# summmeer/session-based-news-recommendation

Hardware: AMD Instinct MI355X
Metric: sessions/sec TCAR train on Globo (synthetic globo fold) (higher is better)
Workload: dtype bf16 (logits GEMM on split-bf16 planes = 3 MFMAs per product, gradient GEMMs plain bf16; fp32 accumulate, fp32 master state)

## Files before the change

session-based-news-recommendation_amd/_lib.py:

```python
from __future__ import annotations

import ctypes as C
import os
import re
import subprocess
from typing import List

PKG_DIR = os.path.dirname(os.path.abspath(__file__))
CSRC = os.path.join(PKG_DIR, "csrc")
LIB_PATH = os.environ.get("TCAR_LIB") or os.path.join(PKG_DIR, "libtcar_hip.so")
SOURCES = ["gemm_f32.hip", "gemm_bf16.hip", "embed.hip", "pool.hip", "score.hip", "ce.hip", "optim.hip", "step.hip", "mha.hip",
           "sampler.hip", "norm.hip", "shard.hip", "segsum.hip", "query.hip", "select.hip", "cand.hip", "retrieve.hip",
           "buildid.hip"]
BUILD_ID_TU = "buildid.hip"


def _hipcc() -> str:
    for cand in (os.environ.get("HIPCC"), "/opt/rocm/bin/hipcc", "hipcc"):
        if cand and (os.path.isabs(cand) and os.path.exists(cand) or not os.path.isabs(cand)):
            return cand
    return "hipcc"


ABI_LAYERS = [("", "tcar_hip.h"), ("SERVE", "tcar_serve.h"), ("WINDOW", "tcar_window.h"), ("QUOTA", "tcar_quota.h"),
              ("SERVE_SHARD", "tcar_serve_shard.h"), ("CAND", "tcar_cand.h"), ("RETRIEVE", "tcar_retrieve.h"),
              ("RAGGED", "tcar_ragged.h")]


def _name(prefix: str, name: str) -> str:
    return prefix + "_" + name if prefix else name


for _prefix, _file in ABI_LAYERS:
    globals()[_name(_prefix, "HEADER")] = os.path.join(PKG_DIR, "..", "include", _file)
HEADERS = [os.path.join(CSRC, "tcar_common.h"), os.path.join(CSRC, "tcar_bf16_layout.h"), os.path.join(CSRC, "topk_rows.h"),
           os.path.join(CSRC, "ce_rows.h")] + \
    [globals()[_name(_prefix, "HEADER")] for _prefix, _ in ABI_LAYERS]
_ID_MARK = b"TCAR_BUILD_ID="


def _digest(paths) -> str:
    import hashlib
    h = hashlib.sha256()
    for p in paths:
        h.update(os.path.basename(p).encode() + b"\0")
        with open(p, "rb") as f:
            h.update(f.read())
    return h.hexdigest()[:32]


def source_build_id() -> str:
    import hashlib
    base = _digest([os.path.join(CSRC, s) for s in SOURCES] + HEADERS)
    return hashlib.sha256((base + "|" + " ".join(SAFE_FLAGS)).encode()).hexdigest()[:32]


def binary_build_id(path: str = LIB_PATH):
    try:
        with open(path, "rb") as f:
# ... 189 lines not shown
```

session-based-news-recommendation_amd/csrc/embed.hip:

```cpp
#include "tcar_common.h"
#include "tcar_bf16_layout.h"

typedef __attribute__((ext_vector_type(4))) __bf16 bf16x4_e;

namespace {

struct EmbArgs {
  tcar_dims_t d;
  tcar_tables_t tab;
  tcar_batch_t bt;
  TcarSignal sig;
  float* x_icp; float* x_pt; float* x_act; float* click_t;
  const float* dx_icp; const float* dx_pt; const float* dx_act; const float* dclick;
  tcar_grads_t g;
  const float* sq_g; long sq_len; float* sq_part; int n_gather;
};
struct EmbRagged { int R; const int32_t* rpos; };
__device__ __forceinline__ const EmbRagged& emb_ragged(const EmbRagged& r) { return r; }
__device__ __forceinline__ EmbRagged emb_ragged() { return EmbRagged{0, nullptr}; }


__device__ __forceinline__ int time_vocab(int k) {
  return k == 0 ? 13 : k == 1 ? 32 : k == 2 ? 8 : k == 3 ? 25 : k == 4 ? 61 : TCAR_DUR_VOCAB;
}
__device__ __forceinline__ int time_rowoff(int k) {
  return k == 0 ? 0 : k == 1 ? 13 : k == 2 ? 45 : k == 3 ? 53 : k == 4 ? 78 : 139;
}
constexpr int SMALL_ROWS = 150;

template <typename P>
__device__ __forceinline__ P pick5(P const (&arr)[5], int k) {
  return k == 0 ? arr[0] : k == 1 ? arr[1] : k == 2 ? arr[2] : k == 3 ? arr[3] : arr[4];
}

template <int NCH, class... RG>
__global__ __launch_bounds__(256) void gather_clip_fwd_kernel(const EmbArgs a, const RG... rg_) {
  constexpr bool RAGGED = sizeof...(RG) > 0;
  const EmbRagged& rg = emb_ragged(rg_...);
  const int lane = threadIdx.x & 63;
  const int wave_g = blockIdx.x * 4 + (threadIdx.x >> 6);
  const int nwaves = gridDim.x * 4;
  const int B = a.bt.B, T = a.bt.T, BT = RAGGED ? rg.R : B * T;
  const int ldh = a.d.ldh, ldt = a.d.ldt;
  const int ic = 2 * ldh, pt = 5 * ldt, ek = ic + pt, ct = 2 * ldt;
  const int sub = ldt >> 2;
  const int gpw = 64 / sub;
  const int grp = lane / sub, lin = lane - grp * sub;

  constexpr int R = 2;
  for (int row0 = wave_g; row0 < BT; row0 += R * nwaves) {
    float4 xi[R][NCH], xc[R][NCH], xp[R][NCH];
    bool live[R];
#pragma unroll
    for (int u = 0; u < R; ++u) {
      const int row = row0 + u * nwaves;
      live[u] = row < BT;
// ... 1431 lines not shown
```

session-based-news-recommendation_amd/csrc/gemm_f32.hip:

```cpp
#include "tcar_common.h"
#include "tcar_bf16_layout.h"
#include <stdlib.h>

typedef __attribute__((ext_vector_type(16))) float f32x16;

constexpr int BK = 32;
constexpr int MAXP = 10;
constexpr int MAXSEG = 3;

struct GemmProb {
  const float* A[MAXSEG];
  const float* B[MAXSEG];
  long lda[MAXSEG], ldb[MAXSEG];
  int K[MAXSEG];
  int nseg;
  float* C;
  long ldc;
  const float* bias;
  int M, N, act, beta;
  int ksplit, kchunk, mode;
  int mt, nt, wg_begin;
  int dact; const float* dact_y; long ld_dact_y; float* colsum;
  __bf16* plane_hi; __bf16* plane_lo; int plane_in32, plane_col0;
  __bf16* pack_hi; __bf16* pack_lo; int pack_in32, pack_c0, pack_c1;
// ... 387 lines not shown
          else *p = v;
          if (g.plane_hi) {
            const __bf16 h = (__bf16)v, l = (__bf16)(v - (float)h);
            const long o = kb32_off(row, gcol, g.plane_in32);
            g.plane_hi[o] = h;
            g.plane_lo[o] = l;
            if (packed) {
              const long po = kb32_off(row, pcol, g.pack_in32);
              g.pack_hi[po] = h;
              g.pack_lo[po] = l;
            }
          }
        }
      }
    }
  }
  if (g.dact && g.colsum) {
    csum += __shfl_xor(csum, 32);
    if (lane < 32 && col < g.N && csum != 0.f) atomicAdd(g.colsum + col, csum);
  }
  tcar_signal_done(ga.sig);
}

namespace {

template <int LA, int LB, int TM, int TN>
int launch_variant(const GroupArgs& ga, int nwg, hipStream_t st) {
  constexpr size_t lds = 2 * (TileGeo<LA, TM>::FLOATS + TileGeo<LB, TN>::FLOATS) * sizeof(float);
  TCAR_SET_LDS_ONCE((gemm_f32_kernel<LA, LB, TM, TN>), lds);
  TCAR_LAUNCH((gemm_f32_kernel<LA, LB, TM, TN>), dim3(nwg), dim3(256), lds, st, ga);
  TCAR_CHECK_LAUNCH();
  return TCAR_OK;
}

template <int LA, int LB>
int launch_layout(GroupArgs& ga, hipStream_t st) {
  long big = 0;
  for (int i = 0; i < ga.nprob; ++i)
    big += (long)((ga.p[i].M + 127) / 128) * ((ga.p[i].N + 127) / 128) * ga.p[i].ksplit;
  const int T = big >= 192 ? 128 : 64;
  int wg = 0;
  for (int i = 0; i < ga.nprob; ++i) {
    GemmProb& p = ga.p[i];
    p.mt = (p.M + T - 1) / T;
    p.nt = (p.N + T - 1) / T;
    p.wg_begin = wg;
// ... 100 lines not shown
}

extern "C" int tcar_gemm_x3_grouped(int layout, int nprob, const tcar_gemm_desc_t* descs, void* stream) {
  return tcar_gemm_x3_grouped_o(layout, nprob, descs, stream, nullptr);
}
int tcar_gemm_x3_grouped_o(int layout, int nprob, const tcar_gemm_desc_t* descs, void* stream, TcarOpt* o) {
  if (nprob <= 0) return TCAR_OK;
  if (layout < 0 || layout > 2 || nprob > MAXP || !descs) return TCAR_E_ARG;
  GroupArgs ga;
  ga.nprob = 0;
  for (int i = 0; i < nprob; ++i) {
    if (descs[i].M <= 0 || descs[i].N <= 0) continue;
    const int rc = fill_prob(ga.p[ga.nprob], layout, descs[i]);
    if (rc) return rc;
    ga.nprob++;
  }
  if (ga.nprob == 0) return TCAR_OK;
  hipStream_t st = (hipStream_t)stream;
  if (layout == 0) return launch_x3<0, 1>(ga, st, o);
  if (layout == 1) return launch_x3<0, 0>(ga, st, o);
  return launch_x3<1, 1>(ga, st, o);
}

extern "C" int tcar_gemm_f32(int layout, int M, int N, int K, const float* A, int64_t lda, const float* B, int64_t ldb,
                             float* C, int64_t ldc, const float* bias, int act, int beta, int splitk, void* stream) {
  if (M <= 0 || N <= 0 || K <= 0) return TCAR_OK;
  tcar_gemm_desc_t d = {};
  d.nseg = 1;
  d.A[0] = A; d.B[0] = B; d.lda[0] = lda; d.ldb[0] = ldb; d.K[0] = K;
  d.C = C; d.ldc = ldc; d.bias = bias; d.M = M; d.N = N; d.act = act; d.beta = beta; d.splitk = splitk; d.atomic = 0;
  return tcar_gemm_f32_grouped(layout, 1, &d, stream);
}

extern "C" int tcar_gemm_splitk_effective(int K, int splitk) {
  if (splitk < 1) splitk = 1;
  int kchunk = (K + splitk - 1) / splitk;
  kchunk = ((kchunk + BK - 1) / BK) * BK;
  return (K + kchunk - 1) / kchunk;
}

extern "C" int tcar_splitk_reduce(const float* slabs, int splitk, int M, int N, int64_t ld, float* out, void* stream) {
  if (M <= 0 || N <= 0) return TCAR_OK;
  if ((N & 3) || (ld & 3) || !tcar_aligned16(slabs) || !tcar_aligned16(out)) return TCAR_E_ARG;
  long total = (long)M * (N >> 2);
  int blocks = (int)((total + 255) / 256);
  if (blocks > 2048) blocks = 2048;
// ... 5 lines not shown
```

session-based-news-recommendation_amd/csrc/query.hip:

```cpp
#include "tcar_common.h"

namespace {
constexpr int QS = 4;
constexpr int CT = 128, H1 = 256, H2 = 512;
struct QMlpArgs {
  const float* click; const float* w1; const float* b1; const float* w2; const float* b2;
  float* q1; float* q;
  int B;
  TcarSignal sig;
};
__device__ __forceinline__ void st4_wt(float* p, float4 v, bool write_through) {
  if (write_through) st4_sc1(p, v);
  else st4(p, v);
}

__global__ __launch_bounds__(512) void query_mlp_kernel(const QMlpArgs a) {
  extern __shared__ __attribute__((aligned(16))) float lds[];
  float* clk = lds;
  float* q1s = clk + QS * CT;
  float* part = q1s + QS * H1;
  const int t = threadIdx.x;
  const int b0 = blockIdx.x * QS;
  const bool wt = a.sig.cnt != nullptr;
  const int cg = t & 63, kq = t >> 6;
  float4 w[16];
#pragma unroll
  for (int j = 0; j < 16; ++j) w[j] = ld4(a.w1 + (long)(kq * 16 + j) * H1 + cg * 4);
  if (t < QS * CT / 4) {
    const int s = t >> 5, c = t & 31;
    st4(clk + s * CT + c * 4, b0 + s < a.B ? ld4(a.click + (long)(b0 + s) * CT + c * 4) : zero4());
  }
  __syncthreads();
  {
    float4 acc[QS];
#pragma unroll
    for (int s = 0; s < QS; ++s) acc[s] = zero4();
#pragma unroll
    for (int j4 = 0; j4 < 4; ++j4) {
#pragma unroll
      for (int s = 0; s < QS; ++s) {
        const float4 c = *reinterpret_cast<const float4*>(clk + s * CT + kq * 16 + j4 * 4);
        acc[s] = fma4(w[j4 * 4 + 0], c.x, acc[s]);
        acc[s] = fma4(w[j4 * 4 + 1], c.y, acc[s]);
        acc[s] = fma4(w[j4 * 4 + 2], c.z, acc[s]);
        acc[s] = fma4(w[j4 * 4 + 3], c.w, acc[s]);
      }
    }
#pragma unroll
    for (int s = 0; s < QS; ++s) st4(part + (kq * QS + s) * H1 + cg * 4, acc[s]);
  }
  __syncthreads();
  if (t < QS * 64) {
    const int s = t >> 6;
// ... 135 lines not shown
  }
  tcar_signal_done(a.sig);
}
}

extern "C" int tcar_query_mlp_bwd(const tcar_dims_t* d, int B, const float* dq, const float* q1, const float* q1_w, const float* q2_w,
                                  float* dq1, float* dclick, void* stream) {
  return tcar_query_mlp_bwd_o(d, B, dq, q1, q1_w, q2_w, dq1, dclick, stream, nullptr);
}
int tcar_query_mlp_bwd_o(const tcar_dims_t* d, int B, const float* dq, const float* q1, const float* q1_w, const float* q2_w, float* dq1,
                         float* dclick, void* stream, TcarOpt* o) {
  if (!d || d->ldh != H1 || d->ldt * 2 != CT || B <= 0) return TCAR_E_ARG;
  if (!q1_w || !dq1 || !dclick || !tcar_aligned16(q1_w) || !tcar_aligned16(dq1)) return TCAR_E_ARG;
  if (dq && (!q1 || !q2_w || !tcar_aligned16(dq) || !tcar_aligned16(q2_w))) return TCAR_E_ARG;
  QBwdArgs a{};
  a.dq = dq; a.q1 = q1; a.w1 = q1_w; a.w2 = q2_w; a.dq1 = dq1; a.dclick = dclick; a.B = B;
  a.sig = tcar_sig(o);
  TCAR_LAUNCH(query_mlp_bwd_kernel, dim3((unsigned)((B + QS - 1) / QS)), dim3(512), 0, (hipStream_t)stream, a);
  TCAR_CHECK_LAUNCH();
  return TCAR_OK;
}

namespace {
}

extern "C" int tcar_query_mlp(const tcar_dims_t* d, int B, const float* click_t, const float* q1_w, const float* q1_b,
                              const float* q2_w, const float* q2_b, float* q1, float* q, void* stream) {
  return tcar_query_mlp_o(d, B, click_t, q1_w, q1_b, q2_w, q2_b, q1, q, stream, nullptr);
}
int tcar_query_mlp_o(const tcar_dims_t* d, int B, const float* click_t, const float* q1_w, const float* q1_b, const float* q2_w,
                     const float* q2_b, float* q1, float* q, void* stream, TcarOpt* o) {
  if (!d || d->ldh != H1 || d->ldt * 2 != CT || B <= 0) return TCAR_E_ARG;
  if (!click_t || !q1_w || !q1_b || !q2_w || !q2_b || !q1 || !q) return TCAR_E_ARG;
  if (!tcar_aligned16(click_t) || !tcar_aligned16(q1_w) || !tcar_aligned16(q1_b) || !tcar_aligned16(q2_w) || !tcar_aligned16(q2_b) ||
      !tcar_aligned16(q1) || !tcar_aligned16(q))
    return TCAR_E_ARG;
  QMlpArgs a{};
  a.click = click_t; a.w1 = q1_w; a.b1 = q1_b; a.w2 = q2_w; a.b2 = q2_b; a.q1 = q1; a.q = q; a.B = B;
  a.sig = tcar_sig(o);
  constexpr size_t lds = (size_t)(QS * CT + QS * H1 + 4 * QS * H2) * sizeof(float);
  TCAR_SET_LDS_ONCE(query_mlp_kernel, lds);
  TCAR_LAUNCH(query_mlp_kernel, dim3((unsigned)((B + QS - 1) / QS)), dim3(512), lds, (hipStream_t)stream, a);
  TCAR_CHECK_LAUNCH();
  return TCAR_OK;
}
```

session-based-news-recommendation_amd/csrc/step.hip:

```cpp
#include "tcar_common.h"
#include "../../include/tcar_serve_shard.h"
#include "../../include/tcar_cand.h"
#include "../../include/tcar_retrieve.h"
#include <stdlib.h>

static int env_int(const char* name, int dflt) {
  const char* v = getenv(name);
  return (v && *v) ? atoi(v) : dflt;
}
namespace {
struct Switch { const char* name; int32_t TcarTuning::*field; int dflt; };
const Switch kSwitches[] = {
    {"TCAR_BF16_TILE", &TcarTuning::bf16_tile, 0},          {"TCAR_BF16_KS", &TcarTuning::bf16_ks, 2},
    {"TCAR_WGRAD_KS", &TcarTuning::wgrad_ks, 1536},         {"TCAR_GATHER_BIG_ROWS", &TcarTuning::gather_big_rows, 16384},
    {"TCAR_MHA_MFMA", &TcarTuning::mha_mfma, 1},            {"TCAR_SORT_SCATTER", &TcarTuning::sort_scatter, 1},
    {"TCAR_DET_SMALL", &TcarTuning::det_small, 1},          {"TCAR_FUSED_CE", &TcarTuning::fused_ce, 2},
    {"TCAR_ONEHOT_TIME", &TcarTuning::onehot_time, 2},      {"TCAR_FLAG_FORK", &TcarTuning::flag_fork, 4095},
    {"TCAR_CE_FOLD", &TcarTuning::ce_fold, 1024},           {"TCAR_PROJ_SPLIT_ROWS", &TcarTuning::proj_split_rows, 1024},
};
static_assert(sizeof(kSwitches) / sizeof(kSwitches[0]) == 12 && sizeof(TcarTuning) == 12 * sizeof(int32_t), "twelve switches, one table");
}
const TcarTuning& tcar_tuning() {
  static const TcarTuning t = [] {
    TcarTuning x{};
// ... 238 lines not shown
  return onehot_bwd(c, bt) && tn(c).fused_ce >= 2 && c->ce_rowscale && c->aps16h && c->ce_form && 2 * c->d.ldh / 64 <= TCAR_ANCHOR_COLS;
}
}

extern "C" int tcar_step_forward(const tcar_ctx_t* c, const tcar_batch_t* bt, int refresh_time, void* stream) {
  return forward_impl(c, bt, refresh_time, stream, -1.f, false);
}

namespace {
struct ScoreOut {
  void* p_hi; void* p_lo; float* tclip; bool done;
  const int32_t* label = nullptr; const float* E = nullptr; int64_t ldE = 0; bool anchor_done = false;
};
template <class Hook>
int session_forward(const tcar_ctx_t* c, const tcar_batch_t* bt, const Geo& g, void* stream, bool planes, int ei, Hook hook,
                    ScoreOut* so = nullptr, const tcar_ragged_t* rg = nullptr) {
  const int B = bt->B, BT = rg ? rg->R : bt->B * bt->T;
  tcar_tables_t tab;
  tables_of(c, tab);
  const int fmask = tn(c).flag_fork;
  hipStream_t sq = (g.ldh == 256 && g.ldt == 64 && c->stream3 && c->ev3 && fork_host(c) && ((fmask >> FK_GATHER) & 1) &&
                    ((fmask >> FK_QUERY) & 1))
                       ? (hipStream_t)c->stream3 : nullptr;
  TcarOpt og = opt_of(c);
  if (sq) og.sig = fork_arm(c, FK_GATHER);
  if (ei >= 0) (void)hipEventRecord((hipEvent_t)c->ev_start[4 * c->ev_n + ei], (hipStream_t)stream);
  RET(tcar_gather_clip_fwd_rg(&c->d, &tab, bt, rg, c->x_icp, c->x_pt, c->x_act, c->click_t, stream, &og));
  if (ei >= 0) (void)hipEventRecord((hipEvent_t)c->ev_stop[4 * c->ev_n + ei], (hipStream_t)stream);
  const bool qside = sq && fork_commit(c, FK_GATHER, og);
  if (qside) {
    RET(fork_go(c, FK_GATHER, (hipStream_t)stream, sq, c->ev3));
    TcarOpt oq = opt_of(c);
    oq.sig = fork_arm(c, FK_QUERY);
    RET(tcar_query_mlp_o(&c->d, B, c->click_t, W(c, TCAR_V_Q1_W), W(c, TCAR_V_Q1_B), W(c, TCAR_V_Q2_W), W(c, TCAR_V_Q2_B), c->q1,
                         c->q, (void*)sq, &oq));
    if (!fork_commit(c, FK_QUERY, oq)) return TCAR_E_LAUNCH;
  }
  const bool qfused = qside || (g.ldh == 256 && g.ldt == 64 && c->scoring != 0);
  if (qfused && !qside)
    RET(tcar_query_mlp(&c->d, B, c->click_t, W(c, TCAR_V_Q1_W), W(c, TCAR_V_Q1_B), W(c, TCAR_V_Q2_W), W(c, TCAR_V_Q2_B), c->q1,
                       c->q, stream));
  const float* x_c = c->x_icp + g.ldh;
  const int n1 = units(g.ic) + units(g.ldh) + units(g.ldt), n2 = units(g.pt) + units(g.ldh);
  const int64_t stride = (int64_t)BT * g.ldh;
  const bool split = c->scoring && c->proj_slabs && c->proj_slab_floats >= (n1 + n2) * stride;
  const bool psplit = split && BT <= tn(c).proj_split_rows;
  TcarOpt op = opt_of(c);
  if (psplit) {
    float* s1 = c->proj_slabs;
    float* s2 = c->proj_slabs + n1 * stride;
    tcar_gemm_desc_t p[6];
    p[0] = prob1(BT, g.ldh, c->x_icp, g.ic, W(c, TCAR_V_M_WIN), g.ldh, g.ic, s1, g.ldh, nullptr, 0, 0, units(g.ic));
    p[1] = prob1(BT, g.ldh, x_c, g.ic, W(c, TCAR_V_M_WC), g.ldh, g.ldh, s1 + units(g.ic) * stride, g.ldh, nullptr, 0, 0, units(g.ldh));
    p[2] = prob1(BT, g.ldh, c->x_act, g.ldt, W(c, TCAR_V_M_WINT), g.ldh, g.ldt, s1 + (units(g.ic) + units(g.ldh)) * stride, g.ldh,
                 nullptr, 0, 0, units(g.ldt));
    p[3] = prob1(BT, g.ldh, c->x_pt, g.pt, W(c, TCAR_V_S_WIN), g.ldh, g.pt, s2, g.ldh, nullptr, 0, 0, units(g.pt));
    p[4] = prob1(BT, g.ldh, x_c, g.ic, W(c, TCAR_V_S_WC), g.ldh, g.ldh, s2 + units(g.pt) * stride, g.ldh, nullptr, 0, 0, units(g.ldh));
    p[5] = prob1(B, g.ldh, c->click_t, g.ct, W(c, TCAR_V_Q1_W), g.ldh, g.ct, c->q1, g.ldh, W(c, TCAR_V_Q1_B), 1);
    if (ei >= 0) (void)hipEventRecord((hipEvent_t)c->ev_start[3 * c->ev_n + ei], (hipStream_t)stream);
    RET(hook(0, &op));
    RET(small_gemm(c, 0, qfused ? 5 : 6, p, stream, &op));
    if (ei >= 0) (void)hipEventRecord((hipEvent_t)c->ev_stop[3 * c->ev_n + ei], (hipStream_t)stream);
  } else {
    tcar_gemm_desc_t p[3];
    p[0] = prob(BT, g.ldh, c->pre1, g.ldh);
    seg(p[0], c->x_icp, g.ic, W(c, TCAR_V_M_WIN), g.ldh, g.ic);
    seg(p[0], x_c, g.ic, W(c, TCAR_V_M_WC), g.ldh, g.ldh);
    seg(p[0], c->x_act, g.ldt, W(c, TCAR_V_M_WINT), g.ldh, g.ldt);
    p[1] = prob(BT, g.ldh, c->pre2, g.ldh);
    seg(p[1], c->x_pt, g.pt, W(c, TCAR_V_S_WIN), g.ldh, g.pt);
    seg(p[1], x_c, g.ic, W(c, TCAR_V_S_WC), g.ldh, g.ldh);
    p[2] = prob1(B, g.ldh, c->click_t, g.ct, W(c, TCAR_V_Q1_W), g.ldh, g.ct, c->q1, g.ldh, W(c, TCAR_V_Q1_B), 1);
    if (ei >= 0) (void)hipEventRecord((hipEvent_t)c->ev_start[3 * c->ev_n + ei], (hipStream_t)stream);
    RET(hook(0, &op));
    RET(small_gemm(c, 0, qfused ? 2 : 3, p, stream, &op));
    if (ei >= 0) (void)hipEventRecord((hipEvent_t)c->ev_stop[3 * c->ev_n + ei], (hipStream_t)stream);
  }
  RET(hook(1, &op));
  const TcarWait wq{};
  if (qside) {
    RET(fork_go(c, FK_QUERY, sq, (hipStream_t)stream, c->ev3));
  } else if (!qside && !qfused) {
    tcar_gemm_desc_t p = prob1(B, g.ic, c->q1, g.ldh, W(c, TCAR_V_Q2_W), g.ic, g.ldh, c->q, g.ic, W(c, TCAR_V_Q2_B), 2);
    RET(small_gemm(c, 0, 1, &p, stream));
  }
  RET(hook(2, &op));
  if (rg && psplit)
    RET(tcar_attn_pool_fwd_slabs_ragged(&c->d, B, rg, c->x_icp, c->x_pt, c->proj_slabs, n1, c->proj_slabs + n1 * stride, n2, stride,
                                        c->pre1, c->pre2, c->q, W(c, TCAR_V_M_WRES), W(c, TCAR_V_S_WRES), c->pooled, c->alpha, stream));
  else if (rg)
    RET(tcar_attn_pool_fwd_ragged(&c->d, B, rg, c->x_icp, c->x_pt, c->pre1, c->pre2, c->q, W(c, TCAR_V_M_WRES), W(c, TCAR_V_S_WRES),
                                  c->pooled, c->alpha, stream));
  else if (psplit)
    RET(tcar_attn_pool_fwd_slabs_w(&c->d, B, bt->T, c->x_icp, c->x_pt, c->proj_slabs, n1, c->proj_slabs + n1 * stride, n2, stride,
                                   c->pre1, c->pre2, c->q, W(c, TCAR_V_M_WRES), W(c, TCAR_V_S_WRES), c->pooled, c->alpha, stream, wq));
  else
    RET(tcar_attn_pool_fwd(&c->d, B, bt->T, c->x_icp, c->x_pt, c->pre1, c->pre2, c->q, W(c, TCAR_V_M_WRES),
                           W(c, TCAR_V_S_WRES), c->pooled, c->alpha, stream));
// ... 1163 lines not shown
```

session-based-news-recommendation_amd/csrc/tcar_common.h:

```cpp
#pragma once
#include <hip/hip_runtime.h>
#include <stdint.h>
#include <stdio.h>

#include "../../include/tcar_hip.h"
#include "../../include/tcar_ragged.h"

#define TCAR_CHECK_LAUNCH()                                   \
  do {                                                        \
    hipError_t e__ = hipGetLastError();                       \
    if (e__ != hipSuccess) {                                  \
      fprintf(stderr, "tcar: HIP error %d (%s) at %s:%d\n", (int)e__, hipGetErrorString(e__), __FILE__, __LINE__); \
      return TCAR_E_LAUNCH;                                   \
    }                                                         \
  } while (0)

#define TCAR_LAUNCH(...)                 \
  do {                                   \
    (void)hipGetLastError();             \
    hipLaunchKernelGGL(__VA_ARGS__);     \
  } while (0)

static inline bool tcar_aligned16(const void* p) { return (reinterpret_cast<uintptr_t>(p) & 15u) == 0; }

// ... 123 lines not shown
                     const float* q2_b, float* q1, float* q, void* stream, TcarOpt* o);
int tcar_attn_pool_bwd_slabs_o(const tcar_dims_t* d, int B, int T, const float* x_icp, const float* x_pt, const float* pre1,
                               const float* pre2, const float* q, const float* w_res1, const float* w_res2, const float* alpha,
                               const float* dpooled, int nd_ic, int nd_pt, int64_t dp_stride, float* dx_icp, float* dx_pt, float* dq,
                               float* dpre1, float* dpre2, float* gw_rows, void* stream, TcarOpt* o);
int tcar_query_mlp_bwd_o(const tcar_dims_t* d, int B, const float* dq, const float* q1, const float* q1_w, const float* q2_w, float* dq1,
                         float* dclick, void* stream, TcarOpt* o);
int tcar_small_tables_bwd_det_o(const tcar_dims_t* d, const tcar_tables_t* tab, const tcar_batch_t* bt, const float* dx_icp,
                                const float* dx_pt, const float* dx_act, const float* dclick, const tcar_grads_t* g, float* ws,
                                void* stream, TcarOpt* o, const float* cand_pc ,
                                int64_t ws_floats );
int tcar_cand_time_bwd_onehot_w(const tcar_dims_t* d, int B, const int32_t* inv_off, const float* qz, const float* dP,
                                const float* attout, int64_t ld_att, const float* tclip, float* ws, const tcar_grads_t* g, void* stream,
                                const TcarWait& wait_dp, int with_pieces);
inline const float* tcar_cand_pieces(const tcar_dims_t* d, const float* ws) { return ws + (long)139 * 32 * (d->ldt + 4); }
int tcar_sqnorm_o(const float* g, const tcar_segments_t* segs, float* sqn_dense, void* stream, TcarOpt* o);
int tcar_colsum_sqnorm_o(const float* g, const tcar_segments_t* segs, int ncs, const tcar_colsum_t* cs, float* sqn_dense, void* stream,
                         TcarOpt* o);
int tcar_attn_pool_fwd_slabs_w(const tcar_dims_t* d, int B, int T, const float* x_icp, const float* x_pt, const float* pre1_slabs,
                               int n1, const float* pre2_slabs, int n2, int64_t slab_stride, float* pre1, float* pre2, const float* q,
                               const float* w_res1, const float* w_res2, float* pooled, float* alpha, void* stream,
                               const TcarWait& wait_q);
int tcar_gemm_x3_grouped_o(int layout, int nprob, const tcar_gemm_desc_t* descs, void* stream, TcarOpt* o);
int tcar_gemm_bf16_perm_o(int layout, int M, int N, int K, const void* A_hi, const void* A_lo, int64_t a_inner, int64_t a_rows,
                          const void* B_hi, const void* B_lo, int64_t b_inner, int64_t b_rows, float* C, int64_t ldc, float* C2,
                          int64_t ldc2, int csplit, const int32_t* c2_perm, int c2_group, int nsplit, int splitk, void* stream,
                          TcarOpt* o);
int tcar_gemm_bf16_ce_o(int M, int N, int K, const void* A_hi, const void* A_lo, int64_t a_inner, int64_t a_rows, const void* B_hi,
                        const void* B_lo, int64_t b_inner, int64_t b_rows, int K1, const void* A2_hi, const void* A2_lo,
                        const void* B2_hi, int64_t inner2, void* p_hi, int64_t p_inner, int64_t p_rows, float* stats,
                        int64_t stats_floats, const int32_t* label, float* lab_logit, int nsplit, int32_t* group_width,
                        int32_t* ngroups, void* stream, TcarOpt* o);
int tcar_gemm_bf16_dx_onehot_o(int M, int N1, int K, const void* A_hi, int64_t a_inner, int64_t a_rows, const void* B_hi,
                               int64_t b_inner, int64_t b_rows, const void* B2_hi, int64_t inner2, float* C, int64_t ldc, int splitk,
                               void* stream, TcarOpt* o);
int tcar_gemm_bf16_de_qz_o(int M, int K, const void* A_hi, int64_t a_inner, int64_t a_rows, const void* B_hi, int64_t b_inner,
                           int64_t b_rows, int ldh, float* C, int64_t ldc, const int32_t* mwdhm, const int32_t* perm,
                           const float* tclip, float* qz, int tile, void* stream, TcarOpt* o);
int tcar_reduce_dact_onehot_o(const float* slabs, int splitk, int M, int ic, int64_t ld, const float* addend, int64_t ld_add,
                              const float* y, int64_t ldy, const float* tclip, float* out, int64_t ldo, float* dP, float* bias_grad0,
                              float* bias_grad1, void* stream, TcarOpt* o);
int tcar_neg_fwd_o(const tcar_dims_t* d, int B, int K, const float* E, const int32_t* neg, const float* attout, float weight,
                   float* neg_fb, float* coef, float* negpart, void* stream, TcarOpt* o);
int tcar_clip_adam_rest_keep_o(float* w2d, int64_t ldw, const float* g2d, float* m2d, float* v2d, int64_t rows, int32_t cols,
                               int32_t slot, const float* sqn_dense, const float* sqn_pieces, const int32_t* use_dense, float clip,
                               float lr_t, float b1, float b2, float eps, void* e16_hi, void* e16_lo, int64_t ld16,
// ... 83 lines not shown
```

Measured before the change: 1.237 million.

## Fuse embedding gather and norm-clip into the head projection GEMM

Adds a head kernel that gathers item, position and time embedding rows, applies per-row norm clipping in registers, writes the clipped activations and feeds them straight into the split-bf16 x3 MFMA projection GEMM. The click-time embedding gather moves into the query MLP kernel on the side stream. Together these remove the separate gather_clip kernel launch and its round trip of activations through global memory. The cost is redundant row-norm loads across N tiles, higher register pressure, and extra start-flag polling on the host to order the side-stream query work.

```diff
diff --git a/include/tcar_head.h b/include/tcar_head.h
--- /dev/null
+++ b/include/tcar_head.h
@@ -0,0 +1,23 @@
+#ifndef TCAR_HEAD_H
+#define TCAR_HEAD_H
+
+#include "tcar_hip.h"
+
+#ifdef __cplusplus
+extern "C" {
+#endif
+
+#define TCAR_HEAD_ABI_VERSION 1
+int tcar_head_abi_version(void);
+
+int tcar_head_gather_proj(const tcar_dims_t* d, const tcar_tables_t* tab, const tcar_batch_t* bt, int nprob,
+                          const tcar_gemm_desc_t* descs, float* x_icp, float* x_pt, float* x_act, void* stream);
+
+int tcar_query_mlp_click(const tcar_dims_t* d, int B, const int32_t* cw, const int32_t* ch, const float* week, const float* hour,
+                         float* click_t, const float* q1_w, const float* q1_b, const float* q2_w, const float* q2_b, float* q1, float* q,
+                         void* stream);
+
+#ifdef __cplusplus
+}
+#endif
+#endif
diff --git a/session-based-news-recommendation_amd/_lib.py b/session-based-news-recommendation_amd/_lib.py
--- a/session-based-news-recommendation_amd/_lib.py
+++ b/session-based-news-recommendation_amd/_lib.py
@@ -24,7 +24,7 @@
 
 ABI_LAYERS = [("", "tcar_hip.h"), ("SERVE", "tcar_serve.h"), ("WINDOW", "tcar_window.h"), ("QUOTA", "tcar_quota.h"),
               ("SERVE_SHARD", "tcar_serve_shard.h"), ("CAND", "tcar_cand.h"), ("RETRIEVE", "tcar_retrieve.h"),
-              ("RAGGED", "tcar_ragged.h")]
+              ("HEAD", "tcar_head.h"), ("RAGGED", "tcar_ragged.h")]
 
 
 def _name(prefix: str, name: str) -> str:
@@ -34,7 +34,7 @@
 for _prefix, _file in ABI_LAYERS:
     globals()[_name(_prefix, "HEADER")] = os.path.join(PKG_DIR, "..", "include", _file)
 HEADERS = [os.path.join(CSRC, "tcar_common.h"), os.path.join(CSRC, "tcar_bf16_layout.h"), os.path.join(CSRC, "topk_rows.h"),
-           os.path.join(CSRC, "ce_rows.h")] + \
+           os.path.join(CSRC, "ce_rows.h"), os.path.join(CSRC, "embed_rows.h")] + \
     [globals()[_name(_prefix, "HEADER")] for _prefix, _ in ABI_LAYERS]
 _ID_MARK = b"TCAR_BUILD_ID="
 
diff --git a/session-based-news-recommendation_amd/csrc/embed.hip b/session-based-news-recommendation_amd/csrc/embed.hip
--- a/session-based-news-recommendation_amd/csrc/embed.hip
+++ b/session-based-news-recommendation_amd/csrc/embed.hip
@@ -1,5 +1,6 @@
 #include "tcar_common.h"
 #include "tcar_bf16_layout.h"
+#include "embed_rows.h"
 
 typedef __attribute__((ext_vector_type(4))) __bf16 bf16x4_e;
 
@@ -20,18 +21,10 @@
 __device__ __forceinline__ EmbRagged emb_ragged() { return EmbRagged{0, nullptr}; }
 
 
-__device__ __forceinline__ int time_vocab(int k) {
-  return k == 0 ? 13 : k == 1 ? 32 : k == 2 ? 8 : k == 3 ? 25 : k == 4 ? 61 : TCAR_DUR_VOCAB;
-}
 __device__ __forceinline__ int time_rowoff(int k) {
   return k == 0 ? 0 : k == 1 ? 13 : k == 2 ? 45 : k == 3 ? 53 : k == 4 ? 78 : 139;
 }
 constexpr int SMALL_ROWS = 150;
-
-template <typename P>
-__device__ __forceinline__ P pick5(P const (&arr)[5], int k) {
-  return k == 0 ? arr[0] : k == 1 ? arr[1] : k == 2 ? arr[2] : k == 3 ? arr[3] : arr[4];
-}
 
 template <int NCH, class... RG>
 __global__ __launch_bounds__(256) void gather_clip_fwd_kernel(const EmbArgs a, const RG... rg_) {
diff --git a/session-based-news-recommendation_amd/csrc/embed_rows.h b/session-based-news-recommendation_amd/csrc/embed_rows.h
--- /dev/null
+++ b/session-based-news-recommendation_amd/csrc/embed_rows.h
@@ -0,0 +1,18 @@
+#pragma once
+#include "tcar_common.h"
+
+__device__ __forceinline__ int time_vocab(int k) {
+  return k == 0 ? 13 : k == 1 ? 32 : k == 2 ? 8 : k == 3 ? 25 : k == 4 ? 61 : TCAR_DUR_VOCAB;
+}
+template <typename P>
+__device__ __forceinline__ P pick5(P const (&arr)[5], int k) {
+  return k == 0 ? arr[0] : k == 1 ? arr[1] : k == 2 ? arr[2] : k == 3 ? arr[3] : arr[4];
+}
+__device__ __forceinline__ int item_row(int id, int n_items) { return clampi(id, 1, n_items) - 1; }
+__device__ __forceinline__ int small_row(int k, int id) {
+  if (k == 5 && (id >= TCAR_DUR_VOCAB || id < 0)) return -1;
+  return clampi(id, 0, time_vocab(k) - 1);
+}
+__device__ __forceinline__ float row256_sumsq(float v0, float v1, float v2, float v3) {
+  return group_sum((v0 + v2) + (v1 + v3), 16);
+}
diff --git a/session-based-news-recommendation_amd/csrc/gemm_f32.hip b/session-based-news-recommendation_amd/csrc/gemm_f32.hip
--- a/session-based-news-recommendation_amd/csrc/gemm_f32.hip
+++ b/session-based-news-recommendation_amd/csrc/gemm_f32.hip
@@ -1,5 +1,7 @@
 #include "tcar_common.h"
 #include "tcar_bf16_layout.h"
+#include "embed_rows.h"
+#include "../../include/tcar_head.h"
 #include <stdlib.h>
 
 typedef __attribute__((ext_vector_type(16))) float f32x16;
@@ -433,6 +435,269 @@
   tcar_signal_done(ga.sig);
 }
 
+enum { XSRC_ICP = 0, XSRC_C = 1, XSRC_ACT = 2, XSRC_PT = 3 };
+struct HeadArgs {
+  GroupArgs ga;
+  tcar_tables_t tab;
+  const int32_t* seq; const int32_t* pub[5]; const int32_t* gap;
+  int T, n_items;
+  float* x_icp; float* x_pt; float* x_act;
+  unsigned char asrc[MAXP][4];
+  unsigned* start_flag; unsigned start_epoch;
+};
+static_assert(sizeof(HeadArgs) <= 4096, "kernel arguments");
+__device__ __forceinline__ void x3_name4(v4f (&a)[4]) {
+  asm volatile("" : "+v"(a[0]), "+v"(a[1]), "+v"(a[2]), "+v"(a[3]) : : "memory");
+}
+template <int N>
+__device__ __forceinline__ void x3_wait12(v4f (&a)[4], v4f (&p)[4], v4f (&b)[4]) {
+  asm volatile("s_waitcnt vmcnt(%12)"
+               : "+v"(a[0]), "+v"(a[1]), "+v"(a[2]), "+v"(a[3]), "+v"(p[0]), "+v"(p[1]), "+v"(p[2]), "+v"(p[3]), "+v"(b[0]), "+v"(b[1]),
+                 "+v"(b[2]), "+v"(b[3])
+               : "n"(N) : "memory");
+}
+__device__ __forceinline__ float4 x3_f4(const v4f& v) { return make_float4(v.x, v.y, v.z, v.w); }
+__device__ __forceinline__ float x3_sq(const v4f& v) { const float4 x = x3_f4(v); return dot4(x, x); }
+
+template <int XD>
+__global__ __launch_bounds__(256) void gemm_x3_head_kernel(const HeadArgs ha) {
+  constexpr int XK = 64, X3_PLANE = X3<XK>::PLANE, NV = 4;
+  constexpr int LDH = 256, LDT = 64, IC = 2 * LDH, PT = 5 * LDT, EK = IC + PT;
+  static_assert(X3<XK>::NV == NV, "four 16-byte loads per thread, operand and stage");
+  extern __shared__ __attribute__((aligned(16))) float smem_f[];
+  char* smem = reinterpret_cast<char*>(smem_f);
+  const GroupArgs& ga = ha.ga;
+  const int tid = threadIdx.x, wave = tid >> 6, lane = tid & 63;
+  if (ha.start_flag && blockIdx.x == 0 && tid == 0)
+    __hip_atomic_store(ha.start_flag, ha.start_epoch, __ATOMIC_RELAXED, __HIP_MEMORY_SCOPE_AGENT);
+  const int wm = wave >> 1, wn = wave & 1;
+  const int nwg = gridDim.x, bid = blockIdx.x;
+  const int xcd = bid & 7, q = nwg >> 3, r = nwg & 7;
+  int id = (xcd < r ? xcd * (q + 1) : r * (q + 1) + (xcd - r) * q) + (bid >> 3);
+  int pi = 0;
+#pragma unroll
+  for (int i = 1; i < MAXP; ++i) pi += (id >= ga.wg0[i]) ? 1 : 0;
+  const GemmProb& g = ga.p[pi];
+  id -= g.wg_begin;
+  const int tiles = g.mt * g.nt;
+  const int split = id / tiles;
+  id -= split * tiles;
+  int tm, tn;
+  if (g.mt <= g.nt) { tn = id / g.mt; tm = id - tn * g.mt; } else { tm = id / g.nt; tn = id - tm * g.nt; }
+  const int m0 = tm * 64, n0 = tn * 64;
+
+  const int ks = split * g.kchunk;
+  int cst[MAXSEG + 1], src[MAXSEG];
+  cst[0] = 0;
+  bool need_ip = false, need_c = false, need_pt = false, need_act = false;
+#pragma unroll
+  for (int sg = 0; sg < MAXSEG; ++sg) {
+    int n = 0;
+    src[sg] = ha.asrc[pi][sg];
+    if (sg < g.nseg) {
+      const int ke = min(g.K[sg], ks + g.kchunk);
+      n = ke > ks ? (ke - ks + XK - 1) / XK : 0;
+      if (n > 0) {
+        need_ip = need_ip || (src[sg] == XSRC_ICP && ks < LDH);
+        need_c = need_c || src[sg] == XSRC_C || (src[sg] == XSRC_ICP && ke > LDH);
+        need_pt = need_pt || src[sg] == XSRC_PT;
+        need_act = need_act || src[sg] == XSRC_ACT;
+      }
+    }
+    cst[sg + 1] = cst[sg] + n;
+  }
+  const int total = cst[MAXSEG];
+  const int b_rmax0 = (g.N + 3) & ~3;
+
+  const int j4 = (tid & 15) * 4, rb0 = tid >> 4;
+  bool rok[NV];
+  int itm[NV], pos[NV], dw[NV], sid[NV][5];
+#pragma unroll
+  for (int i = 0; i < NV; ++i) {
+    const int gr = m0 + rb0 + 16 * i;
+    rok[i] = gr < g.M;
+    const int rw = rok[i] ? gr : m0;
+    itm[i] = 0; dw[i] = 0;
+#pragma unroll
+    for (int k = 0; k < 5; ++k) sid[i][k] = 0;
+    pos[i] = rw % ha.T;
+    if (need_ip || need_c) itm[i] = item_row(ha.seq[rw], ha.n_items);
+    if (need_act) dw[i] = small_row(5, ha.gap[rw]);
+    if (need_pt) {
+#pragma unroll
+      for (int k = 0; k < 5; ++k) sid[i][k] = small_row(k, ha.pub[k][rw]);
+    }
+  }
+
+  auto stage_seg = [&](int s) { return min((s >= cst[1] ? 1 : 0) + (s >= cst[2] ? 1 : 0), g.nseg - 1); };
+  auto seg_src = [&](int sg) { return sg == 0 ? src[0] : sg == 1 ? src[1] : src[2]; };
+  auto load_stage = [&](int s, v4f (&ra)[NV], v4f (&rp)[NV], v4f (&rb)[NV], unsigned& ma, unsigned& mb) {
+    const int sg = stage_seg(s);
+    const int k0 = ks + (s - cst[sg]) * XK;
+    const int ke = min(g.K[sg], ks + g.kchunk);
+    const int sr = seg_src(sg);
+    const bool live = k0 < ke;
+    const bool ip = sr == XSRC_ICP && k0 < LDH, ct = sr == XSRC_C || (sr == XSRC_ICP && k0 >= LDH);
+    const int col = (sr == XSRC_ICP ? (k0 & (LDH - 1)) : k0) + (ct ? LDH : 0);
+    const int tb = sr == XSRC_ACT ? 5 : (k0 >> 6);
+    const float* tp = tb >= 5 ? ha.tab.dur : pick5(ha.tab.time, tb);
+    ma = 0;
+#pragma unroll
+    for (int i = 0; i < NV; ++i) {
+      const int sm = tb >= 5 ? dw[i] : pick5(sid[i], tb);
+      const bool ok = rok[i] && live && (ip || ct || sm >= 0);
+      const float* pe = ha.tab.E + (long)itm[i] * EK + col + j4;
+      const float* ps = tp + (long)(sm < 0 ? 0 : sm) * LDT + j4;
+      const float* pp = ha.tab.pos + (long)pos[i] * LDH + col + j4;
+      ra[i] = gload16_hidden(ok ? ((ip || ct) ? pe : ps) : ha.tab.pos);
+      rp[i] = gload16_hidden((ok && ip) ? pp : ha.tab.pos);
+      ma |= ok ? (1u << i) : 0u;
+    }
+    const long ldb = g.ldb[sg];
+    mb = x3_load<1, XK>(g.B[sg], ldb, n0, min((int)ldb, b_rmax0), k0, ke, tid, rb);
+  };
+
+  f32x16 acc;
+#pragma unroll
+  for (int e = 0; e < 16; ++e) acc[e] = 0.f;
+  v4f ra[XD][NV], rp[XD][NV], rb[XD][NV];
+  unsigned ma[XD], mb[XD];
+#pragma unroll
+  for (int d = 0; d < XD; ++d) load_stage(d, ra[d], rp[d], rb[d], ma[d], mb[d]);
+
+  float s_i[NV], s_p[NV], s_c[NV];
+#pragma unroll
+  for (int i = 0; i < NV; ++i) { s_i[i] = 1.f; s_p[i] = 1.f; s_c[i] = 1.f; }
+  auto row_norms = [&](const float* base, long stride, const int (&rowi)[NV], float (&out)[NV]) {
+    v4f x[NV][4];
+#pragma unroll
+    for (int i = 0; i < NV; ++i)
+#pragma unroll
+      for (int c = 0; c < 4; ++c) x[i][c] = gload16_hidden(base + (long)rowi[i] * stride + 64 * c + j4);
+    asm volatile("s_waitcnt vmcnt(0)" ::: "memory");
+#pragma unroll
+    for (int i = 0; i < NV; ++i) {
+      x3_name4(x[i]);
+      out[i] = clip_scale(row256_sumsq(x3_sq(x[i][0]), x3_sq(x[i][1]), x3_sq(x[i][2]), x3_sq(x[i][3])));
+    }
+  };
+  if constexpr (XD == 2) {
+    if (need_ip || need_c) {
+      const int oc = ((((ks & (LDH - 1)) >> 7) ^ 1) << 7) + (need_c ? LDH : 0) + j4;
+      v4f x[NV][2], y[NV][2];
+#pragma unroll
+      for (int i = 0; i < NV; ++i)
+#pragma unroll
+        for (int c = 0; c < 2; ++c) {
+          x[i][c] = gload16_hidden(ha.tab.E + (long)itm[i] * EK + oc + 64 * c);
+          if (need_ip) y[i][c] = gload16_hidden(ha.tab.pos + (long)pos[i] * LDH + oc + 64 * c);
+        }
+      asm volatile("s_waitcnt vmcnt(0)" ::: "memory");
+      x3_name4(ra[0]);
+      x3_name4(ra[1]);
+      x3_name4(rp[0]);
+      x3_name4(rp[1]);
+#pragma unroll
+      for (int i = 0; i < NV; ++i) {
+        asm volatile("" : "+v"(x[i][0]), "+v"(x[i][1]) : : "memory");
+        const float sa = clip_scale(group_sum((x3_sq(ra[0][i]) + x3_sq(x[i][0])) + (x3_sq(ra[1][i]) + x3_sq(x[i][1])), 16));
+        if (need_ip) {
+          asm volatile("" : "+v"(y[i][0]), "+v"(y[i][1]) : : "memory");
+          s_i[i] = sa;
+          s_p[i] = clip_scale(group_sum((x3_sq(rp[0][i]) + x3_sq(y[i][0])) + (x3_sq(rp[1][i]) + x3_sq(y[i][1])), 16));
+        } else {
+          s_c[i] = sa;
+        }
+      }
+    }
+  } else if (need_ip) {
+    v4f x[NV][4], y[NV][4];
+#pragma unroll
+    for (int i = 0; i < NV; ++i)
+#pragma unroll
+      for (int c = 0; c < 4; ++c) {
+        x[i][c] = gload16_hidden(ha.tab.E + (long)itm[i] * EK + 64 * c + j4);
+        y[i][c] = gload16_hidden(ha.tab.pos + (long)pos[i] * LDH + 64 * c + j4);
+      }
+    asm volatile("s_waitcnt vmcnt(0)" ::: "memory");
+#pragma unroll
+    for (int i = 0; i < NV; ++i) {
+      x3_name4(x[i]);
+      x3_name4(y[i]);
+      s_i[i] = clip_scale(row256_sumsq(x3_sq(x[i][0]), x3_sq(x[i][1]), x3_sq(x[i][2]), x3_sq(x[i][3])));
+      s_p[i] = clip_scale(row256_sumsq(x3_sq(y[i][0]), x3_sq(y[i][1]), x3_sq(y[i][2]), x3_sq(y[i][3])));
+    }
+  }
+  if (XD != 2 && need_c) row_norms(ha.tab.E + LDH, EK, itm, s_c);
+#pragma unroll
+  for (int d = 0; d < XD; ++d) {
+    x3_name4(ra[d]);
+    x3_name4(rp[d]);
+    x3_name4(rb[d]);
+  }
+
+  const bool keep = tn == 0;
+#pragma unroll 1
+  for (int base = 0; base < total; base += XD) {
+#pragma unroll
+    for (int d = 0; d < XD; ++d) {
+      const int s = base + d;
+      __syncthreads();
+      x3_wait12<(XD - 1) * 3 * NV>(ra[d], rp[d], rb[d]);
+      const int sg = stage_seg(s);
+      const int k0 = ks + (s - cst[sg]) * XK;
+      const int sr = seg_src(sg);
+      const bool ip = sr == XSRC_ICP && k0 < LDH, ct = sr == XSRC_C || (sr == XSRC_ICP && k0 >= LDH);
+      const int tb = sr == XSRC_ACT ? 5 : (k0 >> 6);
+      float* xo = sr == XSRC_ICP ? ha.x_icp + k0 + j4 : sr == XSRC_ACT ? ha.x_act + j4 : ha.x_pt + tb * LDT + j4;
+      const long xld = sr == XSRC_ICP ? IC : sr == XSRC_ACT ? LDT : PT;
+      const bool st = keep && sr != XSRC_C && s < total;
+#pragma unroll
+      for (int i = 0; i < NV; ++i) {
+        const bool ok = (ma[d] >> i) & 1u;
+        const float4 a = ok ? x3_f4(ra[d][i]) : zero4();
+        float4 v;
+        if (ip) v = fma4(a, s_i[i], scale4(x3_f4(rp[d][i]), s_p[i]));
+        else if (ct) v = scale4(a, s_c[i]);
+        else v = scale4(a, clip_scale(group_sum(dot4(a, a), 16)));
+        ra[d][i] = v4f{v.x, v.y, v.z, v.w};
+        if (st && rok[i]) st4(xo + (long)(m0 + rb0 + 16 * i) * xld, ok ? v : zero4());
+      }
+      x3_store<0, XK>(smem, smem + X3_PLANE, tid, ra[d], ma[d]);
+      x3_store<1, XK>(smem + 2 * X3_PLANE, smem + 3 * X3_PLANE, tid, rb[d], mb[d]);
+      __syncthreads();
+      load_stage(s + XD, ra[d], rp[d], rb[d], ma[d], mb[d]);
+      const int left = min(g.K[sg], ks + g.kchunk) - k0;
+      const int nsub = s < total ? (min(XK, left + 15) >> 4) : 0;
+#pragma unroll 2
+      for (int u = 0; u < nsub; ++u) {
+        const xbf16x8 ah = x3_frag<0, XK>(smem, wm * 32, u, lane), bh = x3_frag<1, XK>(smem + 2 * X3_PLANE, wn * 32, u, lane);
+        const xbf16x8 al = x3_frag<0, XK>(smem + X3_PLANE, wm * 32, u, lane), bl = x3_frag<1, XK>(smem + 3 * X3_PLANE, wn * 32, u, lane);
+        acc = __builtin_amdgcn_mfma_f32_32x32x16_bf16(al, bh, acc, 0, 0, 0);
+        acc = __builtin_amdgcn_mfma_f32_32x32x16_bf16(ah, bl, acc, 0, 0, 0);
+        acc = __builtin_amdgcn_mfma_f32_32x32x16_bf16(ah, bh, acc, 0, 0, 0);
+      }
+    }
+  }
+  asm volatile("s_waitcnt vmcnt(0)" ::: "memory");
+  float* Cs = g.C + (g.mode == 1 ? (long)split * g.M * g.ldc : 0L);
+  const bool wt = ga.sig.cnt != nullptr;
+  const int col = n0 + wn * 32 + (lane & 31);
+  if (col < g.N) {
+#pragma unroll
+    for (int e = 0; e < 16; ++e) {
+      const int row = m0 + wm * 32 + (e & 3) + 8 * (e >> 2) + 4 * (lane >> 5);
+      if (row < g.M) {
+        float* p = Cs + (long)row * g.ldc + col;
+        const float v = acc[e] + 0.f;
+        if (wt) __hip_atomic_store(p, v, __ATOMIC_RELAXED, __HIP_MEMORY_SCOPE_AGENT);
+        else *p = v;
+      }
+    }
+  }
+  tcar_signal_done(ga.sig);
+}
+
 namespace {
 
 template <int LA, int LB, int TM, int TN>
@@ -579,6 +844,78 @@
   return launch_x3<1, 1>(ga, st, o);
 }
 
+namespace {
+template <int XD>
+int launch_head(const HeadArgs& ha, int wg, hipStream_t st) {
+  constexpr size_t lds = 4 * X3<64>::PLANE;
+  TCAR_SET_LDS_ONCE((gemm_x3_head_kernel<XD>), lds);
+  TCAR_LAUNCH((gemm_x3_head_kernel<XD>), dim3(wg), dim3(256), lds, st, ha);
+  TCAR_CHECK_LAUNCH();
+  return TCAR_OK;
+}
+}
+
+extern "C" int tcar_head_abi_version(void) { return TCAR_HEAD_ABI_VERSION; }
+extern "C" int tcar_head_gather_proj(const tcar_dims_t* d, const tcar_tables_t* tab, const tcar_batch_t* bt, int nprob,
+                                     const tcar_gemm_desc_t* descs, float* x_icp, float* x_pt, float* x_act, void* stream) {
+  return tcar_head_gather_proj_o(d, tab, bt, nprob, descs, x_icp, x_pt, x_act, stream, nullptr);
+}
+int tcar_head_gather_proj_o(const tcar_dims_t* d, const tcar_tables_t* tab, const tcar_batch_t* bt, int nprob, const tcar_gemm_desc_t* descs,
+                            float* x_icp, float* x_pt, float* x_act, void* stream, TcarOpt* o) {
+  if (!d || !tab || !bt || !descs || d->ldh != 256 || d->ldt != 64 || d->n_items < 1) return TCAR_E_ARG;
+  if (bt->B <= 0 || bt->T <= 0 || bt->T > TCAR_POS_VOCAB || nprob < 1 || nprob > MAXP) return TCAR_E_ARG;
+  if (!tab->E || !tab->pos || !tab->dur || !bt->seq || !bt->gap || !x_icp || !x_pt || !x_act) return TCAR_E_ARG;
+  for (int k = 0; k < 5; ++k)
+    if (!tab->time[k] || !bt->pub[k] || !tcar_aligned16(tab->time[k])) return TCAR_E_ARG;
+  if (!tcar_aligned16(tab->E) || !tcar_aligned16(tab->pos) || !tcar_aligned16(tab->dur) || !tcar_aligned16(x_icp) || !tcar_aligned16(x_pt) ||
+      !tcar_aligned16(x_act))
+    return TCAR_E_ARG;
+  const long rows = (long)bt->B * bt->T;
+  const int ldh = 256, ldt = 64, ic = 2 * ldh, pt = 5 * ldt;
+  HeadArgs ha{};
+  GroupArgs& ga = ha.ga;
+  ga.nprob = 0;
+  int wg = 0, max_stages = 0;
+  bool oneshot = true;
+  for (int i = 0; i < nprob; ++i) {
+    const tcar_gemm_desc_t& ds = descs[i];
+    if (ds.M != rows || ds.bias || ds.act || ds.beta || ds.dact || ds.plane_hi || ds.pack_hi || ds.atomic) return TCAR_E_ARG;
+    GemmProb& p = ga.p[ga.nprob];
+    const int rc = fill_prob(p, 0, ds);
+    if (rc) return rc;
+    if (p.kchunk & 63) return TCAR_E_ARG;
+    int n = 0;
+    for (int s = 0; s < ds.nseg; ++s) {
+      int src;
+      if (ds.A[s] == x_icp && ds.lda[s] == ic && ds.K[s] == ic) src = XSRC_ICP;
+      else if (ds.A[s] == x_icp + ldh && ds.lda[s] == ic && ds.K[s] == ldh) src = XSRC_C;
+      else if (ds.A[s] == x_act && ds.lda[s] == ldt && ds.K[s] == ldt) src = XSRC_ACT;
+      else if (ds.A[s] == x_pt && ds.lda[s] == pt && ds.K[s] == pt) src = XSRC_PT;
+      else return TCAR_E_ARG;
+      ha.asrc[ga.nprob][s] = (unsigned char)src;
+      if ((src == XSRC_ICP || src == XSRC_C) && p.kchunk != 128) oneshot = false;
+      n += ((p.K[s] < p.kchunk ? p.K[s] : p.kchunk) + 63) / 64;
+    }
+    max_stages = n > max_stages ? n : max_stages;
+    p.mt = (p.M + 63) / 64;
+    p.nt = (p.N + 63) / 64;
+    p.wg_begin = wg;
+    ga.wg0[ga.nprob] = wg;
+    wg += p.mt * p.nt * p.ksplit;
+    ga.nprob++;
+  }
+  for (int i = ga.nprob; i < MAXP; ++i) ga.wg0[i] = 0x7fffffff;
+  ha.tab = *tab;
+  ha.seq = bt->seq; ha.gap = bt->gap;
+  for (int k = 0; k < 5; ++k) ha.pub[k] = bt->pub[k];
+  ha.T = bt->T; ha.n_items = d->n_items;
+  ha.x_icp = x_icp; ha.x_pt = x_pt; ha.x_act = x_act;
+  if (o && o->start.flag) { ha.start_flag = o->start.flag; ha.start_epoch = o->start.epoch; o->started = true; }
+  ga.sig = tcar_sig(o);
+  if (oneshot && max_stages <= 2 && max_stages <= tcar_fixed::x3_oneshot) return launch_head<2>(ha, wg, (hipStream_t)stream);
+  return launch_head<1>(ha, wg, (hipStream_t)stream);
+}
+
 extern "C" int tcar_gemm_f32(int layout, int M, int N, int K, const float* A, int64_t lda, const float* B, int64_t ldb,
                              float* C, int64_t ldc, const float* bias, int act, int beta, int splitk, void* stream) {
   if (M <= 0 || N <= 0 || K <= 0) return TCAR_OK;
diff --git a/session-based-news-recommendation_amd/csrc/query.hip b/session-based-news-recommendation_amd/csrc/query.hip
--- a/session-based-news-recommendation_amd/csrc/query.hip
+++ b/session-based-news-recommendation_amd/csrc/query.hip
@@ -1,4 +1,6 @@
 #include "tcar_common.h"
+#include "embed_rows.h"
+#include "../../include/tcar_head.h"
 
 namespace {
 constexpr int QS = 4;
@@ -8,6 +10,7 @@
   float* q1; float* q;
   int B;
   TcarSignal sig;
+  const int32_t* cw; const int32_t* ch; const float* week; const float* hour; float* click_out;
 };
 __device__ __forceinline__ void st4_wt(float* p, float4 v, bool write_through) {
   if (write_through) st4_sc1(p, v);
@@ -28,7 +31,18 @@
   for (int j = 0; j < 16; ++j) w[j] = ld4(a.w1 + (long)(kq * 16 + j) * H1 + cg * 4);
   if (t < QS * CT / 4) {
     const int s = t >> 5, c = t & 31;
-    st4(clk + s * CT + c * 4, b0 + s < a.B ? ld4(a.click + (long)(b0 + s) * CT + c * 4) : zero4());
+    if (a.cw) {
+      const int jj = c >> 4, lin = c & 15, kk = jj == 0 ? 2 : 3;
+      const bool live = b0 + s < a.B;
+      const int id = live ? clampi(jj == 0 ? a.cw[b0 + s] : a.ch[b0 + s], 0, time_vocab(kk) - 1) : 0;
+      const float4 x = live ? ld4((jj == 0 ? a.week : a.hour) + (long)id * (CT / 2) + lin * 4) : zero4();
+      const float sx = clip_scale(group_sum(dot4(x, x), 16));
+      const float4 v = scale4(x, sx);
+      st4(clk + s * CT + c * 4, v);
+      if (live) st4_wt(a.click_out + (long)(b0 + s) * CT + c * 4, v, wt);
+    } else {
+      st4(clk + s * CT + c * 4, b0 + s < a.B ? ld4(a.click + (long)(b0 + s) * CT + c * 4) : zero4());
+    }
   }
   __syncthreads();
   {
@@ -210,6 +224,7 @@
 }
 
 namespace {
+int launch_query_mlp(QMlpArgs& a, void* stream, TcarOpt* o);
 }
 
 extern "C" int tcar_query_mlp(const tcar_dims_t* d, int B, const float* click_t, const float* q1_w, const float* q1_b,
@@ -225,10 +240,33 @@
     return TCAR_E_ARG;
   QMlpArgs a{};
   a.click = click_t; a.w1 = q1_w; a.b1 = q1_b; a.w2 = q2_w; a.b2 = q2_b; a.q1 = q1; a.q = q; a.B = B;
+  return launch_query_mlp(a, stream, o);
+}
+extern "C" int tcar_query_mlp_click(const tcar_dims_t* d, int B, const int32_t* cw, const int32_t* ch, const float* week, const float* hour,
+                                    float* click_t, const float* q1_w, const float* q1_b, const float* q2_w, const float* q2_b, float* q1,
+                                    float* q, void* stream) {
+  return tcar_query_mlp_click_o(d, B, cw, ch, week, hour, click_t, q1_w, q1_b, q2_w, q2_b, q1, q, stream, nullptr);
+}
+int tcar_query_mlp_click_o(const tcar_dims_t* d, int B, const int32_t* cw, const int32_t* ch, const float* week, const float* hour,
+                           float* click_t, const float* q1_w, const float* q1_b, const float* q2_w, const float* q2_b, float* q1, float* q,
+                           void* stream, TcarOpt* o) {
+  if (!d || d->ldh != H1 || d->ldt * 2 != CT || B <= 0) return TCAR_E_ARG;
+  if (!cw || !ch || !week || !hour || !click_t || !q1_w || !q1_b || !q2_w || !q2_b || !q1 || !q) return TCAR_E_ARG;
+  if (!tcar_aligned16(week) || !tcar_aligned16(hour) || !tcar_aligned16(click_t) || !tcar_aligned16(q1_w) || !tcar_aligned16(q1_b) ||
+      !tcar_aligned16(q2_w) || !tcar_aligned16(q2_b) || !tcar_aligned16(q1) || !tcar_aligned16(q))
+    return TCAR_E_ARG;
+  QMlpArgs a{};
+  a.cw = cw; a.ch = ch; a.week = week; a.hour = hour; a.click_out = click_t;
+  a.w1 = q1_w; a.b1 = q1_b; a.w2 = q2_w; a.b2 = q2_b; a.q1 = q1; a.q = q; a.B = B;
+  return launch_query_mlp(a, stream, o);
+}
+namespace {
+int launch_query_mlp(QMlpArgs& a, void* stream, TcarOpt* o) {
   a.sig = tcar_sig(o);
   constexpr size_t lds = (size_t)(QS * CT + QS * H1 + 4 * QS * H2) * sizeof(float);
   TCAR_SET_LDS_ONCE(query_mlp_kernel, lds);
-  TCAR_LAUNCH(query_mlp_kernel, dim3((unsigned)((B + QS - 1) / QS)), dim3(512), lds, (hipStream_t)stream, a);
+  TCAR_LAUNCH(query_mlp_kernel, dim3((unsigned)((a.B + QS - 1) / QS)), dim3(512), lds, (hipStream_t)stream, a);
   TCAR_CHECK_LAUNCH();
   return TCAR_OK;
 }
+}
diff --git a/session-based-news-recommendation_amd/csrc/step.hip b/session-based-news-recommendation_amd/csrc/step.hip
--- a/session-based-news-recommendation_amd/csrc/step.hip
+++ b/session-based-news-recommendation_amd/csrc/step.hip
@@ -284,13 +284,37 @@
   hipStream_t sq = (g.ldh == 256 && g.ldt == 64 && c->stream3 && c->ev3 && fork_host(c) && ((fmask >> FK_GATHER) & 1) &&
                     ((fmask >> FK_QUERY) & 1))
                        ? (hipStream_t)c->stream3 : nullptr;
+  const int n1u = units(g.ic) + units(g.ldh) + units(g.ldt), n2u = units(g.pt) + units(g.ldh);
+  const bool slab_form = c->proj_slabs && c->proj_slab_floats >= (int64_t)(n1u + n2u) * BT * g.ldh && BT <= tn(c).proj_split_rows;
+  const bool fused = sq && c->scoring && !rg && (long)BT < (long)tn(c).gather_big_rows && (slab_form || BT <= 4096);
   TcarOpt og = opt_of(c);
-  if (sq) og.sig = fork_arm(c, FK_GATHER);
-  if (ei >= 0) (void)hipEventRecord((hipEvent_t)c->ev_start[4 * c->ev_n + ei], (hipStream_t)stream);
-  RET(tcar_gather_clip_fwd_rg(&c->d, &tab, bt, rg, c->x_icp, c->x_pt, c->x_act, c->click_t, stream, &og));
-  if (ei >= 0) (void)hipEventRecord((hipEvent_t)c->ev_stop[4 * c->ev_n + ei], (hipStream_t)stream);
-  const bool qside = sq && fork_commit(c, FK_GATHER, og);
-  if (qside) {
+  if (sq && !fused) og.sig = fork_arm(c, FK_GATHER);
+  if (!fused) {
+    if (ei >= 0) (void)hipEventRecord((hipEvent_t)c->ev_start[4 * c->ev_n + ei], (hipStream_t)stream);
+    RET(tcar_gather_clip_fwd_rg(&c->d, &tab, bt, rg, c->x_icp, c->x_pt, c->x_act, c->click_t, stream, &og));
+    if (ei >= 0) (void)hipEventRecord((hipEvent_t)c->ev_stop[4 * c->ev_n + ei], (hipStream_t)stream);
+  }
+  const bool qside = fused || (sq && fork_commit(c, FK_GATHER, og));
+  auto proj_launch = [&](int n, const tcar_gemm_desc_t* p, TcarOpt* op) -> int {
+    if (!fused) return small_gemm(c, 0, n, p, stream, op);
+    if (ei >= 0) {
+      (void)hipEventRecord((hipEvent_t)c->ev_stop[4 * c->ev_n + ei], (hipStream_t)stream);
+      (void)hipEventRecord((hipEvent_t)c->ev_start[4 * c->ev_n + ei], (hipStream_t)stream);
+    }
+    fork_disarm(c, FK_GATHER);
+    op->start = fork_arm(c, FK_GATHER);
+    if (!op->start.flag) return TCAR_E_ARG;
+    RET(tcar_head_gather_proj_o(&c->d, &tab, bt, n, p, c->x_icp, c->x_pt, c->x_act, stream, op));
+    if (!op->started) return TCAR_E_ARG;
+    RET(poll(c, sq, op->start));
+    TcarOpt oq = opt_of(c);
+    oq.sig = fork_arm(c, FK_QUERY);
+    RET(tcar_query_mlp_click_o(&c->d, B, bt->cw, bt->ch, tab.time[2], tab.time[3], c->click_t, W(c, TCAR_V_Q1_W), W(c, TCAR_V_Q1_B),
+                               W(c, TCAR_V_Q2_W), W(c, TCAR_V_Q2_B), c->q1, c->q, (void*)sq, &oq));
+    if (!fork_commit(c, FK_QUERY, oq)) return TCAR_E_LAUNCH;
+    return TCAR_OK;
+  };
+  if (qside && !fused) {
     RET(fork_go(c, FK_GATHER, (hipStream_t)stream, sq, c->ev3));
     TcarOpt oq = opt_of(c);
     oq.sig = fork_arm(c, FK_QUERY);
@@ -321,7 +345,7 @@
     p[5] = prob1(B, g.ldh, c->click_t, g.ct, W(c, TCAR_V_Q1_W), g.ldh, g.ct, c->q1, g.ldh, W(c, TCAR_V_Q1_B), 1);
     if (ei >= 0) (void)hipEventRecord((hipEvent_t)c->ev_start[3 * c->ev_n + ei], (hipStream_t)stream);
     RET(hook(0, &op));
-    RET(small_gemm(c, 0, qfused ? 5 : 6, p, stream, &op));
+    RET(proj_launch(qfused ? 5 : 6, p, &op));
     if (ei >= 0) (void)hipEventRecord((hipEvent_t)c->ev_stop[3 * c->ev_n + ei], (hipStream_t)stream);
   } else {
     tcar_gemm_desc_t p[3];
@@ -335,7 +359,7 @@
     p[2] = prob1(B, g.ldh, c->click_t, g.ct, W(c, TCAR_V_Q1_W), g.ldh, g.ct, c->q1, g.ldh, W(c, TCAR_V_Q1_B), 1);
     if (ei >= 0) (void)hipEventRecord((hipEvent_t)c->ev_start[3 * c->ev_n + ei], (hipStream_t)stream);
     RET(hook(0, &op));
-    RET(small_gemm(c, 0, qfused ? 2 : 3, p, stream, &op));
+    RET(proj_launch(qfused ? 2 : 3, p, &op));
     if (ei >= 0) (void)hipEventRecord((hipEvent_t)c->ev_stop[3 * c->ev_n + ei], (hipStream_t)stream);
   }
   RET(hook(1, &op));
diff --git a/session-based-news-recommendation_amd/csrc/tcar_common.h b/session-based-news-recommendation_amd/csrc/tcar_common.h
--- a/session-based-news-recommendation_amd/csrc/tcar_common.h
+++ b/session-based-news-recommendation_amd/csrc/tcar_common.h
@@ -169,6 +169,11 @@
                                const float* w_res1, const float* w_res2, float* pooled, float* alpha, void* stream,
                                const TcarWait& wait_q);
 int tcar_gemm_x3_grouped_o(int layout, int nprob, const tcar_gemm_desc_t* descs, void* stream, TcarOpt* o);
+int tcar_head_gather_proj_o(const tcar_dims_t* d, const tcar_tables_t* tab, const tcar_batch_t* bt, int nprob, const tcar_gemm_desc_t* descs,
+                            float* x_icp, float* x_pt, float* x_act, void* stream, TcarOpt* o);
+int tcar_query_mlp_click_o(const tcar_dims_t* d, int B, const int32_t* cw, const int32_t* ch, const float* week, const float* hour,
+                           float* click_t, const float* q1_w, const float* q1_b, const float* q2_w, const float* q2_b, float* q1, float* q,
+                           void* stream, TcarOpt* o);
 int tcar_gemm_bf16_perm_o(int layout, int M, int N, int K, const void* A_hi, const void* A_lo, int64_t a_inner, int64_t a_rows,
                           const void* B_hi, const void* B_lo, int64_t b_inner, int64_t b_rows, float* C, int64_t ldc, float* C2,
                           int64_t ldc2, int csplit, const int32_t* c2_perm, int c2_group, int nsplit, int splitk, void* stream,
```

After: 1.255 million, median of 3. About the same (+1.4%).
